# theogf/AugmentedGaussianProcesses.jl

Hardware: AMD Instinct MI355X
Metric: cavi_iters_per_sec (higher is better)
Workload: dtype f64

## Files before the change

augmentedgaussianprocesses.jl_amd/csrc/agp_chol.h:

```cpp
#pragma once
#include "agp_cavi.h"
#include "agp_device.h"

namespace agp {

constexpr int LDP = TILE + 2;
#ifndef AGP_PIVOT_ALG
#define AGP_PIVOT_ALG 0
#endif
constexpr int CHOL_THREADS = 512;

__device__ __forceinline__ double rcp1(double p) {
  double r = __builtin_amdgcn_rcp(p);
  return fma(r, fma(-p, r, 1.0), r);
}
__device__ __forceinline__ double rsqrt1(double p) {
  double y = __builtin_amdgcn_rsq(p);
  const double h = 0.5 * p;
  y = y * fma(-h * y, y, 1.5);
  y = y * fma(-h * y, y, 1.5);
  return y;
}
__device__ __forceinline__ float rsqrt1(float p) {
  float y = __builtin_amdgcn_rsqf(p);
  const float h = 0.5f * p;
  y = y * fmaf(-h * y, y, 1.5f);
  return y;
}
__device__ __forceinline__ float rcp1(float p) {
  float r = __builtin_amdgcn_rcpf(p);
  return fmaf(r, fmaf(-p, r, 1.0f), r);
}

template <typename T, int NT>
__device__ __forceinline__ void load_tile_lds(const T* __restrict__ G, int64_t ld, T* S) {
  typedef typename Mfma<T>::vec_t vec_t;
  constexpr int VEC = Mfma<T>::VEC, NV = TILE / VEC;
#pragma unroll
  for (int v = 0; v < TILE * NV / NT; ++v) {
    int vi = threadIdx.x + v * NT;
    int r = vi / NV, cv = vi % NV;
    vec_t x = *reinterpret_cast<const vec_t*>(G + (int64_t)r * ld + cv * VEC);
#pragma unroll
    for (int e = 0; e < VEC; ++e) S[r * LDP + cv * VEC + e] = x[e];
  }
}

template <typename T>
struct Acc8 {
  typename Mfma<T>::acc_t a[2];
  __device__ __forceinline__ void zero() {
#pragma unroll
    for (int i = 0; i < 2; ++i)
#pragma unroll
      for (int r = 0; r < 4; ++r) a[i][r] = T(0);
  }
};

template <typename T>
__device__ __forceinline__ void mma8(const T* As, const T* Bs, Acc8<T>& acc) {
  const int lane = threadIdx.x & 63, wave = threadIdx.x >> 6, wm = wave >> 2, wn = wave & 3;
#pragma unroll 4
  for (int kk = 0; kk < TILE / 4; ++kk) {
    T a0 = As[(wm * 32 + (lane & 15)) * LDP + kk * 4 + (lane >> 4)];
    T a1 = As[(wm * 32 + 16 + (lane & 15)) * LDP + kk * 4 + (lane >> 4)];
    T b0 = Bs[(wn * 16 + (lane & 15)) * LDP + kk * 4 + (lane >> 4)];
    acc.a[0] = Mfma<T>::mma(a0, b0, acc.a[0]);
    acc.a[1] = Mfma<T>::mma(a1, b0, acc.a[1]);
  }
}

template <typename T>
__device__ __forceinline__ void mma8_sub(const T* As, const T* Bs, Acc8<T>& acc) {
  const int lane = threadIdx.x & 63, wave = threadIdx.x >> 6, wm = wave >> 2, wn = wave & 3;
#pragma unroll 4
  for (int kk = 0; kk < TILE / 4; ++kk) {
    T a0 = -As[(wm * 32 + (lane & 15)) * LDP + kk * 4 + (lane >> 4)];
    T a1 = -As[(wm * 32 + 16 + (lane & 15)) * LDP + kk * 4 + (lane >> 4)];
    T b0 = Bs[(wn * 16 + (lane & 15)) * LDP + kk * 4 + (lane >> 4)];
    acc.a[0] = Mfma<T>::mma(a0, b0, acc.a[0]);
    acc.a[1] = Mfma<T>::mma(a1, b0, acc.a[1]);
  }
}

template <typename T, typename F>
__device__ __forceinline__ void acc8_foreach(Acc8<T>& acc, F f) {
  const int lane = threadIdx.x & 63, wave = threadIdx.x >> 6, wm = wave >> 2, wn = wave & 3;
#pragma unroll
  for (int mi = 0; mi < 2; ++mi)
#pragma unroll
    for (int r = 0; r < 4; ++r) {
      T t = acc.a[mi][r];
      f(wm * 32 + mi * 16 + Mfma<T>::row(lane, r), wn * 16 + (lane & 15), t);
      acc.a[mi][r] = t;
    }
}

template <typename T>
__device__ __forceinline__ void mma_lds64(const T* As, const T* Bs, Acc<T>& acc) {
  const int lane = threadIdx.x & 63, wave = threadIdx.x >> 6, wm = wave >> 1, wn = wave & 1;
#pragma unroll 4
  for (int kk = 0; kk < TILE / 4; ++kk) {
    T a0 = As[(wm * 32 + (lane & 15)) * LDP + kk * 4 + (lane >> 4)];
    T a1 = As[(wm * 32 + 16 + (lane & 15)) * LDP + kk * 4 + (lane >> 4)];
    T b0 = Bs[(wn * 32 + (lane & 15)) * LDP + kk * 4 + (lane >> 4)];
    T b1 = Bs[(wn * 32 + 16 + (lane & 15)) * LDP + kk * 4 + (lane >> 4)];
    acc.a[0][0] = Mfma<T>::mma(a0, b0, acc.a[0][0]);
    acc.a[0][1] = Mfma<T>::mma(a0, b1, acc.a[0][1]);
    acc.a[1][0] = Mfma<T>::mma(a1, b0, acc.a[1][0]);
    acc.a[1][1] = Mfma<T>::mma(a1, b1, acc.a[1][1]);
  }
}

constexpr int SC_ELEMS = 2 * 2 * 4 * TILE;

struct NoHook {
  __device__ __forceinline__ void operator()(int) const {}
};

template <typename T, int J, int NS, typename H, int PIV = 0>
__device__ __forceinline__ void chol_rounds(T (&a)[NS][NS], T (&g)[NS][NS], T* sc, T* piv, const bool act, const int ti,
                                            const int tj, H& hook, const int hbase) {
#pragma unroll 1
  for (int rr = 0; rr < 4; ++rr) {
    const int jj0 = rr * 4, j0 = J * 16 + jj0;
    T* P = sc + (rr & 1) * 4 * TILE;
    T* Mw = sc + 2 * 4 * TILE + (rr & 1) * 4 * TILE;
    if (act && PIV != 4) {
      const int qc = tj - jj0, qr = ti - jj0;
      if (qc >= 0 && qc < 4) {
#pragma unroll
        for (int r = J; r < NS; ++r) {
          T v = a[r][J];
          if (r == J) v = (ti >= jj0) ? v : T(0);
          P[qc * TILE + ti + 16 * r] = v;
        }
      }
      if (qr >= 0 && qr < 4) {
#pragma unroll
        for (int c = 0; c <= J; ++c) Mw[qr * TILE + tj + 16 * c] = g[J][c];
      }
    }
    __syncthreads();
    hook(hbase + rr);
    if (!act) continue;
    if (PIV == 4 || PIV == 5) continue;
    const T d00 = P[j0], d10 = P[j0 + 1], d20 = P[j0 + 2], d30 = P[j0 + 3];
    T d11 = P[TILE + j0 + 1], d21 = P[TILE + j0 + 2], d31 = P[TILE + j0 + 3];
    T d22 = P[2 * TILE + j0 + 2], d32 = P[2 * TILE + j0 + 3], d33 = P[3 * TILE + j0 + 3];
    T r0, r1, r2, r3, l10, l20, l30, l21, l31, l32;
    if (PIV == 2) {
      r0 = r1 = r2 = r3 = T(1);
      l10 = d10;
      l20 = d20;
      l30 = d30;
      l21 = d21;
      l31 = d31;
      l32 = d32;
    } else if (PIV == 1) {
      r0 = rcp1(d00);
      const T n11 = fma(d00, d11, -(d10 * d10)), n21 = fma(d00, d21, -(d20 * d10)), n31 = fma(d00, d31, -(d30 * d10));
      const T n22 = fma(d00, d22, -(d20 * d20)), n32 = fma(d00, d32, -(d30 * d20)), n33 = fma(d00, d33, -(d30 * d30));
      const T rm2 = rcp1(n11);
      const T p22 = fma(n11, n22, -(n21 * n21)) * r0, p32 = fma(n11, n32, -(n31 * n21)) * r0;
      const T p33 = fma(n11, n33, -(n31 * n31)) * r0;
      const T rm3 = rcp1(p22);
      const T m4 = fma(p22, p33, -(p32 * p32)) * rm2;
      const T rm4 = rcp1(m4);
      l10 = d10 * r0;
      l20 = d20 * r0;
      l30 = d30 * r0;
      l21 = n21 * rm2;
      l31 = n31 * rm2;
      l32 = p32 * rm3;
      r1 = d00 * rm2;
      r2 = n11 * rm3;
      r3 = p22 * rm4;
      d11 = n11 * r0;
      d22 = p22 * rm2;
      d33 = m4 * rm3;
    } else {
      r0 = rcp1(d00);
      l10 = d10 * r0;
      l20 = d20 * r0;
      l30 = d30 * r0;
      d11 = fma(-l10, d10, d11);
      d21 = fma(-l20, d10, d21);
      d31 = fma(-l30, d10, d31);
      d22 = fma(-l20, d20, d22);
      d32 = fma(-l30, d20, d32);
      d33 = fma(-l30, d30, d33);
      r1 = rcp1(d11);
      l21 = d21 * r1;
      l31 = d31 * r1;
      d22 = fma(-l21, d21, d22);
      d32 = fma(-l31, d21, d32);
      d33 = fma(-l31, d31, d33);
      r2 = rcp1(d22);
      l32 = d32 * r2;
      d33 = fma(-l32, d32, d33);
// ... 76 lines not shown
  const int ti = (tid & 255) >> 4, tj = tid & 15;
  NoHook nohook;
  T a[4][4], g[4][4];
#pragma unroll
  for (int r = 0; r < 4; ++r)
#pragma unroll
    for (int c = 0; c < 4; ++c) {
      int R = ti + 16 * r, Cc = tj + 16 * c;
      int lo = R >= Cc ? R : Cc, hi = R >= Cc ? Cc : R;
      a[r][c] = bufA[lo * LDP + hi];
      g[r][c] = (R == Cc) ? T(1) : T(0);
    }
  __syncthreads();
  chol_rounds<T, 0, 4, NoHook>(a, g, sc, piv, act, ti, tj, nohook, 0);
  chol_rounds<T, 1, 4, NoHook>(a, g, sc, piv, act, ti, tj, nohook, 0);
  chol_rounds<T, 2, 4, NoHook>(a, g, sc, piv, act, ti, tj, nohook, 0);
  chol_rounds<T, 3, 4, NoHook>(a, g, sc, piv, act, ti, tj, nohook, 0);
  __syncthreads();
  if (tid < TILE) {
    const T p = piv[tid];
    const bool bad = !(p > T(0)) && (col0 + tid) < nvalid;
    const unsigned long long mask = __ballot(bad);
    if (mask != 0ull && tid == 0) {
      int32_t want = (int32_t)(col0 + (__ffsll((long long)mask) - 1) + 1);
      int32_t old = atomicCAS(info, 0, want);
      while (old != 0 && old > want) {
        int32_t prev = atomicCAS(info, old, want);
        if (prev == old) break;
        old = prev;
      }
    }
  }
  if (act) {
    T rsC[4], rsR[4];
#pragma unroll
    for (int q = 0; q < 4; ++q) {
      T pc = piv[tj + 16 * q], pr = piv[ti + 16 * q];
      rsC[q] = rsqrt1(pc > T(0) ? pc : T(1));
      rsR[q] = rsqrt1(pr > T(0) ? pr : T(1));
    }
#pragma unroll
    for (int r = 0; r < 4; ++r)
#pragma unroll
      for (int c = 0; c < 4; ++c) {
        int R = ti + 16 * r, Cc = tj + 16 * c;
        bufA[R * LDP + Cc] = (R >= Cc) ? a[r][c] * rsC[c] : T(0);
        bufB[R * LDP + Cc] = (R >= Cc) ? g[r][c] * rsR[r] : T(0);
      }
  }
  __syncthreads();
}

template <typename T, bool TB, int LDB = LDP>
__device__ __forceinline__ typename Mfma<T>::acc_t mma_blk32(const T* As, const T* Bs, typename Mfma<T>::acc_t acc,
                                                             int wr, int wc, int lane, bool negA) {
#pragma unroll
  for (int kk = 0; kk < 8; ++kk) {
    T a = As[(wr * 16 + (lane & 15)) * LDP + kk * 4 + (lane >> 4)];
    if (negA) a = -a;
    T b = TB ? Bs[(kk * 4 + (lane >> 4)) * LDB + wc * 16 + (lane & 15)]
             : Bs[(wc * 16 + (lane & 15)) * LDB + kk * 4 + (lane >> 4)];
    acc = Mfma<T>::mma(a, b, acc);
  }
  return acc;
}

template <typename T, typename H, int PIV = 0>
__device__ __forceinline__ void elim_block32(T* bufA, T* bufB, int o, T* sc, T* piv, const bool act, const int ti,
                                             const int tj, H& hook) {
  T a[2][2], g[2][2];
#pragma unroll
  for (int r = 0; r < 2; ++r)
#pragma unroll
    for (int c = 0; c < 2; ++c) {
      int R = ti + 16 * r, Cc = tj + 16 * c;
      int lo = R >= Cc ? R : Cc, hi = R >= Cc ? Cc : R;
      a[r][c] = bufA[(o + lo) * LDP + o + hi];
      g[r][c] = (R == Cc) ? T(1) : T(0);
    }
  __syncthreads();
  chol_rounds<T, 0, 2, H, PIV>(a, g, sc, piv + o, act, ti, tj, hook, 0);
  chol_rounds<T, 1, 2, H, PIV>(a, g, sc, piv + o, act, ti, tj, hook, 4);
  __syncthreads();
  if (act) {
    T rsC[2], rsR[2];
#pragma unroll
    for (int q = 0; q < 2; ++q) {
      T pc = piv[o + tj + 16 * q], pr = piv[o + ti + 16 * q];
      rsC[q] = rsqrt1(pc > T(0) ? pc : T(1));
      rsR[q] = rsqrt1(pr > T(0) ? pr : T(1));
    }
#pragma unroll
    for (int r = 0; r < 2; ++r)
#pragma unroll
      for (int c = 0; c < 2; ++c) {
        int R = ti + 16 * r, Cc = tj + 16 * c;
        bufA[(o + R) * LDP + o + Cc] = (R >= Cc) ? a[r][c] * rsC[c] : T(0);
        bufB[(o + R) * LDP + o + Cc] = (R >= Cc) ? g[r][c] * rsR[r] : T(0);
      }
  }
  __syncthreads();
}

template <typename T, typename H, int PIV = AGP_PIVOT_ALG>
__device__ __forceinline__ void factor_diag_tile_2lvl(T* bufA, T* bufB, T* sc, T* piv, int32_t* info, int64_t col0,
                                                      int64_t nvalid, H& hook) {
  const int tid = threadIdx.x;
  const bool act = tid < 256;
  const int ti = (tid & 255) >> 4, tj = tid & 15;
  const int lane = tid & 63, wave = tid >> 6, wr = (wave >> 1) & 1, wc = wave & 1;
  const bool mw = wave < 4;
  typedef typename Mfma<T>::acc_t acc_t;
  NoHook nohook;
  elim_block32<T, NoHook, PIV>(bufA, bufB, 0, sc, piv, act, ti, tj, nohook);
  acc_t acc;
#pragma unroll
  for (int r = 0; r < 4; ++r) acc[r] = T(0);
  if (mw) {
    acc = mma_blk32<T, false>(bufA + 32 * LDP, bufB, acc, wr, wc, lane, false);
#pragma unroll
    for (int r = 0; r < 4; ++r)
      bufB[(32 + wr * 16 + Mfma<T>::row(lane, r)) * LDP + wc * 16 + (lane & 15)] = acc[r];
  } else {
    for (int e = tid - 256; e < 32 * 32; e += (int)blockDim.x - 256) {
      bufA[(e >> 5) * LDP + 32 + (e & 31)] = T(0);
      bufB[(e >> 5) * LDP + 32 + (e & 31)] = T(0);
    }
  }
  __syncthreads();
  if (mw) {
#pragma unroll
    for (int r = 0; r < 4; ++r)
      bufA[(32 + wr * 16 + Mfma<T>::row(lane, r)) * LDP + wc * 16 + (lane & 15)] = acc[r];
    if (wr >= wc) {
#pragma unroll
      for (int r = 0; r < 4; ++r)
        acc[r] = bufA[(32 + wr * 16 + Mfma<T>::row(lane, r)) * LDP + 32 + wc * 16 + (lane & 15)];
      acc = mma_blk32<T, false>(bufB + 32 * LDP, bufB + 32 * LDP, acc, wr, wc, lane, true);
#pragma unroll
      for (int r = 0; r < 4; ++r)
        bufA[(32 + wr * 16 + Mfma<T>::row(lane, r)) * LDP + 32 + wc * 16 + (lane & 15)] = acc[r];
    }
  }
  __syncthreads();
  elim_block32<T, H, PIV>(bufA, bufB, 32, sc, piv, act, ti, tj, hook);
#pragma unroll
  for (int r = 0; r < 4; ++r) acc[r] = T(0);
  if (mw) {
    acc = mma_blk32<T, true>(bufA + 32 * LDP, bufB, acc, wr, wc, lane, false);
#pragma unroll
    for (int r = 0; r < 4; ++r) sc[(wr * 16 + Mfma<T>::row(lane, r)) * 32 + wc * 16 + (lane & 15)] = acc[r];
  }
  __syncthreads();
#pragma unroll
  for (int r = 0; r < 4; ++r) acc[r] = T(0);
  if (mw) {
    acc = mma_blk32<T, true, 32>(bufB + 32 * LDP + 32, sc, acc, wr, wc, lane, true);
#pragma unroll
    for (int r = 0; r < 4; ++r) bufB[(32 + wr * 16 + Mfma<T>::row(lane, r)) * LDP + wc * 16 + (lane & 15)] = acc[r];
  }
  if (blockDim.x <= 256) {
    for (int e = tid; e < 32 * 32; e += blockDim.x) {
      bufA[(e >> 5) * LDP + 32 + (e & 31)] = T(0);
      bufB[(e >> 5) * LDP + 32 + (e & 31)] = T(0);
    }
  }
  if (tid < TILE) {
    const T p = piv[tid];
    const bool bad = !(p > T(0)) && (col0 + tid) < nvalid;
    const unsigned long long mask = __ballot(bad);
    if (mask != 0ull && tid == 0) {
      int32_t want = (int32_t)(col0 + (__ffsll((long long)mask) - 1) + 1);
      int32_t old = atomicCAS(info, 0, want);
      while (old != 0 && old > want) {
        int32_t prev = atomicCAS(info, old, want);
        if (prev == old) break;
        old = prev;
      }
    }
  }
  __syncthreads();
}

template <typename T>
__device__ __forceinline__ void factor_diag_tile_2lvl(T* bufA, T* bufB, T* sc, T* piv, int32_t* info, int64_t col0,
                                                      int64_t nvalid) {
  NoHook nohook;
  factor_diag_tile_2lvl<T, NoHook>(bufA, bufB, sc, piv, info, col0, nvalid, nohook);
}

__device__ __forceinline__ double lane_bcast(double v, int l) {
  const int lo = __builtin_amdgcn_readlane(__double2loint(v), l), hi = __builtin_amdgcn_readlane(__double2hiint(v), l);
  return __hiloint2double(hi, lo);
}
__device__ __forceinline__ float lane_bcast(float v, int l) {
  return __int_as_float(__builtin_amdgcn_readlane(__float_as_int(v), l));
}

template <typename T, bool NN>
__device__ __forceinline__ typename Mfma<T>::acc_t mma16(const T* Ar, const T* sa, const T* Bp, int kend,
                                                         typename Mfma<T>::acc_t acc, bool neg, int lane) {
  const int lr = lane & 15, lk = lane >> 4;
  typename Mfma<T>::acc_t p1;
#pragma unroll
  for (int r = 0; r < 4; ++r) p1[r] = T(0);
#pragma unroll 2
  for (int kk = 0; kk < kend; kk += 8) {
    T a0 = Ar[lr * LDP + kk + lk], a1 = Ar[lr * LDP + kk + 4 + lk];
    if (sa) {
      a0 *= sa[kk + lk];
      a1 *= sa[kk + 4 + lk];
    }
    if (neg) {
      a0 = -a0;
      a1 = -a1;
    }
    const T b0 = NN ? Bp[(kk + lk) * LDP + lr] : Bp[lr * LDP + kk + lk];
    const T b1 = NN ? Bp[(kk + 4 + lk) * LDP + lr] : Bp[lr * LDP + kk + 4 + lk];
    acc = Mfma<T>::mma(a0, b0, acc);
    p1 = Mfma<T>::mma(a1, b1, p1);
  }
#pragma unroll
  for (int r = 0; r < 4; ++r) acc[r] += p1[r];
  return acc;
}

template <typename T>
__device__ __forceinline__ typename Mfma<T>::acc_t acc_load16(const T* P, int lane) {
  typename Mfma<T>::acc_t acc;
#pragma unroll
  for (int r = 0; r < 4; ++r) acc[r] = P[Mfma<T>::row(lane, r) * LDP + (lane & 15)];
  return acc;
}
template <typename T>
__device__ __forceinline__ void acc_store16(T* P, typename Mfma<T>::acc_t acc, int lane) {
#pragma unroll
  for (int r = 0; r < 4; ++r) P[Mfma<T>::row(lane, r) * LDP + (lane & 15)] = acc[r];
}

template <typename T, typename H, int CUT = 0>
__device__ __forceinline__ void factor_diag_tile_panel(T* bufA, T* bufB, T* sc, T* piv, int32_t* info, int64_t col0,
                                                       int64_t nvalid, H& hook) {
  const int tid = threadIdx.x, lane = tid & 63, wave = tid >> 6;
  T* rinv = sc;
  T* rs = sc + TILE;
  typedef typename Mfma<T>::acc_t acc_t;
#pragma unroll 1
  for (int s = 0; s < 4; ++s) {
    const int c0 = 16 * s;
    if (wave == 0 && CUT != 2) {
      T a[16], dv[16], rv[16];
#pragma unroll
      for (int c = 0; c < 16; ++c) a[c] = bufA[lane * LDP + c0 + c];
#pragma unroll
      for (int j = 0; j < 16; ++j) {
        const T d = lane_bcast(a[j], c0 + j);
        const T r = rcp1(d);
        const T l = a[j] * r;
        bufA[lane * LDP + c0 + j] = a[j];
        dv[j] = d;
        rv[j] = r;
#pragma unroll
        for (int c = j + 1; c < 16; ++c) a[c] = fma(-l, lane_bcast(a[j], c0 + c), a[c]);
      }
// ... 651 lines not shown
  __builtin_amdgcn_fence(__ATOMIC_RELEASE, "workgroup");
  __syncthreads();
  if (threadIdx.x == 0) __hip_atomic_fetch_add(sync.done, 1, __ATOMIC_RELAXED, __HIP_MEMORY_SCOPE_AGENT);
}

__global__ void k_handshake(int32_t* mine, const int32_t* theirs, int32_t* ok) {
  if (threadIdx.x != 0) return;
  __hip_atomic_store(mine, 1, __ATOMIC_RELAXED, __HIP_MEMORY_SCOPE_SYSTEM);
  long spins = 0;
  int seen = 0;
  while (!(seen = __hip_atomic_load(theirs, __ATOMIC_RELAXED, __HIP_MEMORY_SCOPE_SYSTEM)) && ++spins < 4000) __builtin_amdgcn_s_sleep(16);
  *ok = seen;
}

__global__ void k_wait_ge(const int32_t* __restrict__ p, int32_t want, int32_t* __restrict__ info) {
  if (threadIdx.x != 0) return;
  long spins = 0;
  while ((int32_t)(__hip_atomic_load(p, __ATOMIC_RELAXED, __HIP_MEMORY_SCOPE_SYSTEM) - want) < 0) {
    __builtin_amdgcn_s_sleep(127);
    if (++spins > (1L << 24)) {
      atomicExch(info, -2);
      break;
    }
  }
}

__global__ void k_wait_ge_fast(const int32_t* __restrict__ p, int32_t want, int32_t* __restrict__ info) {
  if (threadIdx.x != 0) return;
  long spins = 0;
  while ((int32_t)(__hip_atomic_load(p, __ATOMIC_RELAXED, __HIP_MEMORY_SCOPE_SYSTEM) - want) < 0) {
    __builtin_amdgcn_s_sleep(8);
    if (++spins > (1L << 27)) {
      atomicExch(info, -2);
      break;
    }
  }
}

__device__ __forceinline__ void dag_signal(int32_t* flag, int32_t epoch) {
  __builtin_amdgcn_fence(__ATOMIC_RELEASE, "workgroup");
  __syncthreads();
  if (threadIdx.x == 0) __hip_atomic_store(flag, epoch, __ATOMIC_RELAXED, __HIP_MEMORY_SCOPE_AGENT);
}

template <typename T>
__device__ __forceinline__ typename Mfma<T>::acc_t mma_tile16(const T* Ar, const T* Bc, int kend,
                                                              typename Mfma<T>::acc_t acc, bool neg, int lane) {
  const T* pa = Ar + (lane & 15) * LDP + (lane >> 4);
  const T* pb = Bc + (lane & 15) * LDP + (lane >> 4);
  typename Mfma<T>::acc_t p1;
#pragma unroll
  for (int r = 0; r < 4; ++r) p1[r] = T(0);
#pragma unroll 2
  for (int kk = 0; kk < kend / 4; kk += 2) {
    T a0 = pa[kk * 4], a1 = pa[kk * 4 + 4];
    const T b0 = pb[kk * 4], b1 = pb[kk * 4 + 4];
    if (neg) {
      a0 = -a0;
      a1 = -a1;
    }
    acc = Mfma<T>::mma(a0, b0, acc);
    p1 = Mfma<T>::mma(a1, b1, p1);
  }
#pragma unroll
  for (int r = 0; r < 4; ++r) acc[r] += p1[r];
  return acc;
}

template <typename T>
struct ChainPrefetch {
  const T* src;
  T *dT, *dD;
  int* bad;
  const int32_t *f1, *f2;
  int32_t epoch;
  int* ok;
  const T* dgsrc;
  T* gDg;
  const T* lsrc;
  T* gL;
  int ld_i;
  bool coh = false;
  T v[TILE * TILE / 256];
  __device__ __forceinline__ void operator()(int round) {
    int t = (int)threadIdx.x - 256;
    if (t < 0) return;
    if (sizeof(T) == 8) asm volatile("" : "+v"(t));
    if (round < 2) {
      if (dgsrc) {
#pragma unroll
        for (int q = 0; q < TILE * TILE / 512; ++q) {
          const int e = t + (2 * q + round) * 256;
          if (coh) __hip_atomic_store(gDg + e, dgsrc[(e >> 6) * LDP + (e & 63)], __ATOMIC_RELAXED, __HIP_MEMORY_SCOPE_AGENT);
          else gDg[e] = dgsrc[(e >> 6) * LDP + (e & 63)];
        }
      }
      return;
    }
    if (round < 4 && lsrc) {
#pragma unroll
      for (int q = 0; q < TILE * TILE / 512; ++q) {
        const int e = t + (2 * q + (round - 2)) * 256;
        gL[(e >> 6) * ld_i + (e & 63)] = lsrc[(e >> 6) * LDP + (e & 63)];
      }
    }
    if (!src) return;
    if (round == 3) {
      if (t == 0)
        *ok = (__hip_atomic_load(f1, __ATOMIC_RELAXED, __HIP_MEMORY_SCOPE_AGENT) == epoch) &&
              (__hip_atomic_load(f2, __ATOMIC_RELAXED, __HIP_MEMORY_SCOPE_AGENT) == epoch);
      return;
    }
    if (round < 4 || round > 6 || !*ok) return;
    if (round >= 5) {
      T* d = round == 5 ? dT : dD;
#pragma unroll
      for (int q = 0; q < TILE * TILE / 256; ++q) {
        const int e = t + q * 256;
        if (is_sent<T>(v[q])) *bad = 1;
        d[(e >> 6) * LDP + (e & 63)] = v[q];
      }
    }
    if (round <= 5) {
      const T* g = round == 4 ? src : src + TILE * TILE;
#pragma unroll
      for (int q = 0; q < TILE * TILE / 256; ++q)
        v[q] = __hip_atomic_load(g + t + q * 256, __ATOMIC_RELAXED, __HIP_MEMORY_SCOPE_AGENT);
    }
  }
};

typedef unsigned int u32x4 __attribute__((ext_vector_type(4)));
__device__ __forceinline__ u32x4 load16_sc1(const void* p) {
  u32x4 v;
  asm volatile("global_load_dwordx4 %0, %1, off sc1" : "=v"(v) : "v"(p) : "memory");
  return v;
}
__device__ __forceinline__ void wait_vmcnt0() { asm volatile("s_waitcnt vmcnt(0)" ::: "memory"); }
template <typename T>
__device__ __forceinline__ T vec16_elem(u32x4 v, int i);
template <>
__device__ __forceinline__ double vec16_elem<double>(u32x4 v, int i) {
  const unsigned long long u = ((unsigned long long)v[2 * i + 1] << 32) | v[2 * i];
  return __builtin_bit_cast(double, u);
}
template <>
__device__ __forceinline__ float vec16_elem<float>(u32x4 v, int i) {
  return __builtin_bit_cast(float, (unsigned int)v[i]);
}
template <typename T>
__device__ __forceinline__ int pro_slot_off(int tid, int e) {
  constexpr int VEC = 16 / (int)sizeof(T);
  return (e / VEC) * (CHOL_THREADS * VEC) + tid * VEC + (e % VEC);
}

template <typename T>
struct EpiArgs {
  int on = 0;
  int64_t B = 0;
  int nslices = 0;
  const T* pk = nullptr;
  int64_t ldp = 0;
  T kdiag = T(0);
  const T* kd_ptr = nullptr;
  int use_kt = 0;
  T jitter = T(0), rho = T(0);
  LikParams<T> lp{};
  const T* y = nullptr;
  const int64_t* idx = nullptr;
  T *Kt = nullptr, *muf = nullptr, *varf = nullptr, *cb = nullptr, *theta = nullptr, *r = nullptr, *w = nullptr;
  int* flags = nullptr;
  const T* lam = nullptr;
  T* gamma = nullptr;
};

template <typename T>
struct ProArgs {
  const T* kap = nullptr;
  int64_t ldk = 0, Kdim = 0;
  const T* w = nullptr;
  const T* r = nullptr;
  T* eta2 = nullptr;
  const T* Kinv = nullptr;
  int64_t ldm = 0;
  T* eta1 = nullptr;
  const T* kinv_mu0 = nullptr;
  T lr = T(0);
  T* HS = nullptr;
  int32_t* sflags = nullptr;
  T* fill = nullptr;
  int64_t fill_n = 0;
  int32_t nfill = 0;
  const T* packed = nullptr;
// ... 54 lines not shown
    __syncthreads();
  }
}

constexpr int ARRIVE_STRIDE = 16;
__device__ __forceinline__ void pro_arrival_gate(const int32_t* arrive, int g, int32_t want, int32_t* info) {
  if (threadIdx.x == 0) {
    long spins = 0;
    while ((int32_t)(__hip_atomic_load(arrive + g * ARRIVE_STRIDE, __ATOMIC_RELAXED, __HIP_MEMORY_SCOPE_AGENT) - want) < 0) {
      __builtin_amdgcn_s_sleep(8);
      if (++spins > (1L << 23)) {
        atomicExch(info, -4);
        break;
      }
    }
  }
  __syncthreads();
  __builtin_amdgcn_fence(__ATOMIC_ACQUIRE, "agent");
}

constexpr int PRO_NEAR = 4;
__host__ __device__ __forceinline__ int64_t pro_nhelp(int64_t nt, int64_t c, int ks, int kf) {
  const int64_t ntc = nt - c, nn = ntc < PRO_NEAR ? ntc : PRO_NEAR;
  return nn * (kf - 1) + (ntc - nn) * (ks - 1);
}
template <typename T>
__device__ __forceinline__ void pro_slice(const T* __restrict__ kap, int64_t ldk, const T* __restrict__ w, int64_t R0, int64_t c0,
                                          int64_t q0, int64_t q1, T* sm, Acc8<T>& acc) {
  constexpr int Q = TILE * TILE / CHOL_THREADS;
  const int r = threadIdx.x & 63, kb = threadIdx.x >> 6;
  const bool dg = R0 == c0;
  T va[Q], vb[Q], wv[Q];
  auto ldg = [&](int64_t qc) {
    const T* __restrict__ p = kap + (qc * TILE) * ldk;
#pragma unroll
    for (int q = 0; q < Q; ++q) {
      const int k = kb + 8 * q;
      va[q] = p[k * ldk + R0 + r];
      vb[q] = dg ? T(0) : p[k * ldk + c0 + r];
      wv[q] = w[qc * TILE + k];
    }
  };
  if (q0 < q1) ldg(q0);
  int cur = 0;
  for (int64_t qc = q0; qc < q1; ++qc) {
    T* As = sm + cur * 2 * TILE * LDP;
    T* Bs = As + TILE * LDP;
#pragma unroll
    for (int q = 0; q < Q; ++q) {
      const int k = kb + 8 * q;
      As[r * LDP + k] = va[q] * wv[q];
      Bs[r * LDP + k] = dg ? va[q] : vb[q];
    }
    __syncthreads();
    if (qc + 1 < q1) ldg(qc + 1);
    mma8<T>(As, Bs, acc);
    cur ^= 1;
  }
  __syncthreads();
}

constexpr long long CHAIN_GO_TICKS = 4LL * 100000000LL;
#ifndef AGP_TILES_WAVES_F64
#define AGP_TILES_WAVES_F64 4
#endif
#ifndef AGP_TILES_WAVES_F32
#define AGP_TILES_WAVES_F32 6
#endif
template <typename T, int ROLE, bool PRO>
constexpr int dag_min_waves() {
  return ROLE != 2 ? 1 : PRO ? (sizeof(T) == 8 ? 2 : 4) : (sizeof(T) == 8 ? AGP_TILES_WAVES_F64 : AGP_TILES_WAVES_F32);
}
template <typename T>
struct ProdArgs {
  T* out = nullptr;
  int64_t ld = 0;
  int64_t base = 0;
  T* fill = nullptr;
  int64_t fill_n = 0;
  double* ld_out = nullptr;
  int32_t* status = nullptr;
};

constexpr int STRACE_SLOTS = 8192, STRACE_XPUB = 600, STRACE_EXT = 1100, STRACE_FILL0 = 1400, STRACE_FILL1 = 1500, STRACE_WG0 = 2048,
              STRACE_WG1 = 4096, STRACE_MAXWG = 2048, STRACE_SAFE0 = 6144, STRACE_SAFE1 = 6400;
#ifdef AGP_STEP_TRACE
struct StraceExit {
  unsigned long long* p;
  __device__ ~StraceExit() {
    if (p && threadIdx.x == 0) *p = wall_clock64();
  }
};
#define STRACE(i) \
  if (PRO && ROLE == 0 && trace && threadIdx.x == 0) trace[i] = wall_clock64()
#else
#define STRACE(i)
#endif

template <typename T, bool FUSED, bool BATCH = false, bool TRACE = false, bool STEP = false, bool PRO = false, int ROLE = 0>
__global__ __launch_bounds__(CHOL_THREADS, (dag_min_waves<T, ROLE, PRO>()))
void k_chol_dag(CholBatch<T> bt, int nb, int64_t fstride, int64_t ld, int64_t ldx,
                                                           int64_t lde, int64_t ne, int64_t nt,
                                                           int32_t* __restrict__ info, int64_t nvalid, int32_t* flags,
                                                           int32_t epoch, unsigned long long* trace, T* H, int64_t hstride,
                                                           int64_t nx_, const T* __restrict__ erow, int opts, DagSync sync,
                                                           ProArgs<T> pro = ProArgs<T>{}, EpiArgs<T> epi = EpiArgs<T>{},
                                                           ProdArgs<T> prod = ProdArgs<T>{}) {
  static_assert(!PRO || (FUSED && !BATCH), "the prologue exists for single-problem launches with a chain workgroup only");
  static_assert(ROLE == 0 || (FUSED && STEP && !TRACE), "the split launch exists for the CAVI step's launches");
  const int64_t nx = STEP ? 0 : nx_;
  const int write_x = STEP ? 0 : (opts & 1);
  const bool store_l = STEP ? false : (opts & 2) != 0;
  const int prob = BATCH ? (int)(blockIdx.x % (unsigned)nb) : 0;
  const int64_t bidx = BATCH ? (int64_t)(blockIdx.x / (unsigned)nb) : (int64_t)blockIdx.x;
  T* A = bt.A[prob];
  T* X = bt.X[prob];
  T* __restrict__ Dg = bt.Dg[prob];
  T* E = bt.E[prob];
  if (BATCH) erow = bt.R[prob];
  flags += prob * fstride;
  constexpr int64_t SLOT = TILE * TILE;
  T* HX = H + prob * hstride;
  T* HP = HX + nt * SLOT;
  T* HL = HP + 2 * nt * SLOT;
  __shared__ __attribute__((aligned(16))) T sm[((FUSED && ROLE != 2) || PRO ? 4 : 2) * TILE * LDP];
  __shared__ __attribute__((aligned(16))) T sc[(ROLE == 2 && !PRO) ? TILE : SC_ELEMS];
  __shared__ T piv[TILE];
  __shared__ int wait_ok, pf_ok, pf_bad;
  if (ROLE == 1) {
    if (threadIdx.x == 0) {
      wait_ok = 1;
      if (sync.here) __hip_atomic_fetch_add(sync.here, 1, __ATOMIC_RELAXED, __HIP_MEMORY_SCOPE_SYSTEM);
      unsigned spins = 0;
      const long long t0 = (long long)wall_clock64();
      while (sync.go) {
        const int32_t d = (int32_t)(__hip_atomic_load(sync.go, __ATOMIC_RELAXED, __HIP_MEMORY_SCOPE_SYSTEM) - sync.go_val);
        if (d == 0) break;
        if (d > 0) {
          wait_ok = 0;
          break;
        }
        __builtin_amdgcn_s_sleep(4);
        if ((++spins & 1023u) == 0 && (long long)wall_clock64() - t0 > CHAIN_GO_TICKS) {
          atomicExch(info, -1);
          wait_ok = 0;
#ifdef AGP_DEBUG_PTRS
          atomicAdd(&agp_dag_diag[5], 1ull);
#endif
          break;
        }
      }
    }
    __syncthreads();
    if (!wait_ok) {
      chain_count_out(sync);
      return;
    }
    __builtin_amdgcn_fence(__ATOMIC_ACQUIRE, "agent");
  }
  T* bufA = sm;
  T* bufB = sm + TILE * LDP;
  const int tid = threadIdx.x;
#ifdef AGP_STEP_TRACE
  StraceExit strace_exit{(PRO && ROLE == 0 && trace && bidx < STRACE_MAXWG) ? trace + STRACE_WG1 + bidx : nullptr};
  if (bidx < STRACE_MAXWG) STRACE(STRACE_WG0 + bidx);
#endif
// ... 251 lines not shown
      acc8_foreach<T>(acc, [&](int r, int cc, T& val) {
        pro.eta2[(R * TILE + r) * pro.ldm + c0 + cc] = val;
        pro.eta2[(c0 + cc) * pro.ldm + R * TILE + r] = val;
        val *= T(-2);
      });
    }
    PRO_TS(tsb + 4);
  } else if (idr) {
    const bool on_diag = (R - nt - ne) == c;
    acc8_foreach<T>(acc, [&](int r, int cc, T& val) { val = (on_diag && r == cc) ? T(1) : T(0); });
  } else if (PRO && ext && R == nt + ne - 1) {
    if (pro.tred && pro.arrive) pro_arrival_gate(pro.arrive, 0, pro.arrive_want, info);
    const int col = tid & 63, grp = tid >> 6;
    T s0 = T(0), s1 = T(0), s2 = T(0), s3 = T(0);
    int64_t k = grp;
    for (; k + 24 < pro.Kdim; k += 32) {
      const T a0 = pro.kap[k * pro.ldk + c0 + col], a1 = pro.kap[(k + 8) * pro.ldk + c0 + col];
      const T a2 = pro.kap[(k + 16) * pro.ldk + c0 + col], a3 = pro.kap[(k + 24) * pro.ldk + c0 + col];
      s0 += a0 * pro.r[k];
      s1 += a1 * pro.r[k + 8];
      s2 += a2 * pro.r[k + 16];
      s3 += a3 * pro.r[k + 24];
    }
    for (; k < pro.Kdim; k += 8) s0 += pro.kap[k * pro.ldk + c0 + col] * pro.r[k];
    sc[grp * TILE + col] = (s0 + s1) + (s2 + s3);
    __syncthreads();
    if (grp == 0) {
      T t = T(0);
#pragma unroll
      for (int q = 0; q < CHOL_THREADS / 64; ++q) t += sc[q * TILE + col];
      if (pro.tred) t = pro.tred[c0 + col];
      T e = pro.eta1[c0 + col];
      e += pro.lr * (t + (pro.kinv_mu0 ? pro.kinv_mu0[c0 + col] : T(0)) - e);
      pro.eta1[c0 + col] = e;
      sc[CHOL_THREADS + col] = e;
    }
    __syncthreads();
    acc8_foreach<T>(acc, [&](int r, int cc, T& val) { val = r == 0 ? sc[CHOL_THREADS + cc] : T(0); });
    __syncthreads();
  } else if (erow && ext && R == nt + ne - 1) {
    acc8_foreach<T>(acc, [&](int r, int cc, T& val) { val = r == 0 ? erow[c0 + cc] : T(0); });
  } else {
    acc8_foreach<T>(acc, [&](int r, int cc, T& val) { val = rowp[r * ldr + c0 + cc]; });
  }
  if (PRO && ROLE == 2 && chain) {
    T* park = HP + SLOT;
    acc8_foreach<T>(acc, [&](int r, int cc, T& val) {
      __hip_atomic_store(park + r * TILE + cc, val, __ATOMIC_RELAXED, __HIP_MEMORY_SCOPE_AGENT);
    });
    dag_signal(pre2, epoch);
    return;
  }
  if (ROLE != 2 && chain) {
    if (PRO && ROLE == 1) {
      if (!dag_wait(pre2, nullptr, epoch, abortf, info, &wait_ok)) {
        chain_count_out(sync);
        return;
      }
      load_tile_lds_hv<T>(HP + SLOT, bufA);
    } else {
      acc8_foreach<T>(acc, [&](int r, int cc, T& val) { bufA[r * LDP + cc] = val; });
    }
    __syncthreads();
    T* bufC = sm + (FUSED ? 2 : 0) * TILE * LDP;
    T* bufD = sm + (FUSED ? 3 : 0) * TILE * LDP;
    for (int64_t k = 0; k < nt; ++k) {
      const int64_t k0 = k * TILE;
      T* trow = A + (k + 1) * TILE * ld;
      ChainPrefetch<T> pf;
      pf.src = k + 1 < nt ? HP + 2 * (k + 1) * SLOT : nullptr;
      pf.bad = &pf_bad;
      pf.dT = bufC;
      pf.dD = bufD;
      pf.f1 = pre1 + (k + 1) * DAG_FS;
      pf.f2 = pre2 + (k + 1) * DAG_FS;
      pf.epoch = epoch;
      pf.ok = &pf_ok;
      pf.dgsrc = k >= 1 ? bufD : nullptr;
      pf.gDg = Dg + (k - 1) * TILE * TILE;
      pf.lsrc = (k >= 1 && store_l) ? bufC : nullptr;
      pf.gL = A + k0 * ld + (k0 - TILE);
      pf.ld_i = (int)ld;
      pf.coh = ROLE == 1;
      if (tid == 0) pf_ok = pf_bad = 0;
      factor_diag_tile_2lvl<T, ChainPrefetch<T>>(bufA, bufB, sc, piv, info, k0, nvalid, pf);
      DAG_TRC(k, 2);
      PRO_TS(512 + k);
      {
        T xv[TILE * TILE / CHOL_THREADS];
        int tl = tid;
        asm volatile("" : "+v"(tl));
#pragma unroll
        for (int q = 0; q < TILE * TILE / CHOL_THREADS; ++q) {
          const int e = tl + q * CHOL_THREADS;
          xv[q] = bufB[(e >> 6) * LDP + (e & 63)];
        }
#pragma unroll
        for (int q = 0; q < TILE * TILE / CHOL_THREADS; ++q) {
          const int e = tl + q * CHOL_THREADS;
          __hip_atomic_store(HX + k * SLOT + e, xv[q], __ATOMIC_RELAXED, __HIP_MEMORY_SCOPE_AGENT);
          if (write_x) X[(k0 + (e >> 6)) * ldx + k0 + (e & 63)] = xv[q];
        }
      }
      if (k + 1 == nt) {
        for (int e = tid; e < TILE * TILE; e += CHOL_THREADS) {
          if (ROLE == 1) __hip_atomic_store(Dg + k * TILE * TILE + e, bufA[(e >> 6) * LDP + (e & 63)], __ATOMIC_RELAXED, __HIP_MEMORY_SCOPE_AGENT);
          else Dg[k * TILE * TILE + e] = bufA[(e >> 6) * LDP + (e & 63)];
        }
        dag_signal(xready + k * DAG_FS, epoch);
        DAG_TRC(k, 3);
        STRACE(STRACE_XPUB);
        if (ROLE == 1) chain_count_out(sync);
        return;
      }
      const bool late_feed = !pf_ok || pf_bad;
      if (late_feed) {
        dag_signal(xready + k * DAG_FS, epoch);
        DAG_TRC(k, 3);
        if (!dag_wait(pf.f1, pf.f2, epoch, abortf, info, &wait_ok)) {
          if (ROLE == 1) chain_count_out(sync);
          return;
        }
        load_tiles_lds_hv2<T>(HP + 2 * (k + 1) * SLOT, bufC, HP + (2 * (k + 1) + 1) * SLOT, bufD);
        __syncthreads();
      }
      if (TRACE && tid == 0) trace[chain_slot(k + 1, nt, ne, nx) * 8 + 7] = (unsigned long long)pf_ok;
      DAG_TRC(k + 1, 4);
      typedef typename Mfma<T>::acc_t acc_t;
      const int lane = tid & 63, wave = tid >> 6;
      {
        const int ri = wave >> 1, cA = (wave & 1) ? 2 : 3, cB = 3 - cA;
        acc_t oa, ob;
#pragma unroll
        for (int r = 0; r < 4; ++r) oa[r] = ob[r] = T(0);
        oa = mma_tile16<T>(bufC + 16 * ri * LDP, bufB + 16 * cA * LDP, 16 * (cA + 1), oa, false, lane);
        ob = mma_tile16<T>(bufC + 16 * ri * LDP, bufB + 16 * cB * LDP, 16 * (cB + 1), ob, false, lane);
        if (!late_feed) {
          dag_signal(xready + k * DAG_FS, epoch);
          DAG_TRC(k, 3);
        } else {
          __syncthreads();
        }
#pragma unroll
        for (int r = 0; r < 4; ++r) {
          const int row = 16 * ri + Mfma<T>::row(lane, r);
          bufC[row * LDP + 16 * cA + (lane & 15)] = oa[r];
          bufC[row * LDP + 16 * cB + (lane & 15)] = ob[r];
          T* hl = HL + ((k + 1) * nt + k) * SLOT + row * TILE + (lane & 15);
          __hip_atomic_store(hl + 16 * cA, oa[r], __ATOMIC_RELAXED, __HIP_MEMORY_SCOPE_AGENT);
          __hip_atomic_store(hl + 16 * cB, ob[r], __ATOMIC_RELAXED, __HIP_MEMORY_SCOPE_AGENT);
        }
      }
      __syncthreads();
      DAG_TRC(k + 1, 5);
      {
        const int ti_[10] = {0, 1, 1, 2, 2, 2, 3, 3, 3, 3}, tj_[10] = {0, 0, 1, 0, 1, 2, 0, 1, 2, 3};
#pragma unroll
        for (int rep = 0; rep < 2; ++rep) {
          const int tl = rep == 0 ? 2 + wave : wave;
          if (rep == 1 && wave >= 2) break;
          int i2 = 0, j2 = 0;
#pragma unroll
          for (int q = 0; q < 10; ++q)
            if (q == tl) {
              i2 = ti_[q];
              j2 = tj_[q];
// ... 210 lines not shown
```

Measured before the change: 3259.

## Overlap L21*X11 glue MMA with second diagonal elimination via idle waves

Moves the L21·X11 product that followed the second 32x32 elimination block into a hook run by the otherwise idle waves 4-7 during a chosen elimination round. The accumulator is written to scratch once the rounds finish, which removes a serial MMA phase and one block barrier from the diagonal-tile factorization. It also drops a redundant zero-fill branch, hardcodes the thread stride, and adds optional step-trace timestamps. The upper waves now carry both the prefetch work and the MMA, which may add register pressure and contention in the rounds.

Measured after the change: 3289 (median of 6 runs). Within noise of the previous version (+0.9%).

```diff
diff --git a/augmentedgaussianprocesses.jl_amd/csrc/agp_chol.h b/augmentedgaussianprocesses.jl_amd/csrc/agp_chol.h
--- a/augmentedgaussianprocesses.jl_amd/csrc/agp_chol.h
+++ b/augmentedgaussianprocesses.jl_amd/csrc/agp_chol.h
@@ -7,6 +7,9 @@
 constexpr int LDP = TILE + 2;
 #ifndef AGP_PIVOT_ALG
 #define AGP_PIVOT_ALG 0
+#endif
+#ifndef AGP_GLUE_ROUND
+#define AGP_GLUE_ROUND 2
 #endif
 constexpr int CHOL_THREADS = 512;
 
@@ -115,7 +118,10 @@
 constexpr int SC_ELEMS = 2 * 2 * 4 * TILE;
 
 struct NoHook {
+  static constexpr int glue_round = 0;
   __device__ __forceinline__ void operator()(int) const {}
+  __device__ __forceinline__ void after_rounds() const {}
+  __device__ __forceinline__ void stamp(int) const {}
 };
 
 template <typename T, int J, int NS, typename H, int PIV = 0>
@@ -358,6 +364,7 @@
   chol_rounds<T, 0, 2, H, PIV>(a, g, sc, piv + o, act, ti, tj, hook, 0);
   chol_rounds<T, 1, 2, H, PIV>(a, g, sc, piv + o, act, ti, tj, hook, 4);
   __syncthreads();
+  hook.after_rounds();
   if (act) {
     T rsC[2], rsR[2];
 #pragma unroll
@@ -377,6 +384,31 @@
   }
   __syncthreads();
 }
+
+template <typename T, typename H>
+struct GlueP {
+  typedef typename Mfma<T>::acc_t acc_t;
+  H& inner;
+  const T *L21, *X11;
+  T* sc;
+  acc_t acc;
+  __device__ __forceinline__ GlueP(H& h, const T* l21, const T* x11, T* s) : inner(h), L21(l21), X11(x11), sc(s) {
+#pragma unroll
+    for (int r = 0; r < 4; ++r) acc[r] = T(0);
+  }
+  __device__ __forceinline__ void operator()(int round) {
+    inner(round);
+    const int tid = threadIdx.x, lane = tid & 63, wave = tid >> 6, wr = (wave >> 1) & 1, wc = wave & 1;
+    if (round == H::glue_round && wave >= 4) acc = mma_blk32<T, true>(L21, X11, acc, wr, wc, lane, false);
+  }
+  __device__ __forceinline__ void after_rounds() {
+    const int tid = threadIdx.x, lane = tid & 63, wave = tid >> 6, wr = (wave >> 1) & 1, wc = wave & 1;
+    if (wave >= 4) {
+#pragma unroll
+      for (int r = 0; r < 4; ++r) sc[(wr * 16 + Mfma<T>::row(lane, r)) * 32 + wc * 16 + (lane & 15)] = acc[r];
+    }
+  }
+};
 
 template <typename T, typename H, int PIV = AGP_PIVOT_ALG>
 __device__ __forceinline__ void factor_diag_tile_2lvl(T* bufA, T* bufB, T* sc, T* piv, int32_t* info, int64_t col0,
@@ -388,7 +420,9 @@
   const bool mw = wave < 4;
   typedef typename Mfma<T>::acc_t acc_t;
   NoHook nohook;
+  hook.stamp(0);
   elim_block32<T, NoHook, PIV>(bufA, bufB, 0, sc, piv, act, ti, tj, nohook);
+  hook.stamp(1);
   acc_t acc;
 #pragma unroll
   for (int r = 0; r < 4; ++r) acc[r] = T(0);
@@ -398,12 +432,13 @@
     for (int r = 0; r < 4; ++r)
       bufB[(32 + wr * 16 + Mfma<T>::row(lane, r)) * LDP + wc * 16 + (lane & 15)] = acc[r];
   } else {
-    for (int e = tid - 256; e < 32 * 32; e += (int)blockDim.x - 256) {
+    for (int e = tid - 256; e < 32 * 32; e += CHOL_THREADS - 256) {
       bufA[(e >> 5) * LDP + 32 + (e & 31)] = T(0);
       bufB[(e >> 5) * LDP + 32 + (e & 31)] = T(0);
     }
   }
   __syncthreads();
+  hook.stamp(2);
   if (mw) {
 #pragma unroll
     for (int r = 0; r < 4; ++r)
@@ -419,27 +454,16 @@
     }
   }
   __syncthreads();
-  elim_block32<T, H, PIV>(bufA, bufB, 32, sc, piv, act, ti, tj, hook);
-#pragma unroll
-  for (int r = 0; r < 4; ++r) acc[r] = T(0);
-  if (mw) {
-    acc = mma_blk32<T, true>(bufA + 32 * LDP, bufB, acc, wr, wc, lane, false);
-#pragma unroll
-    for (int r = 0; r < 4; ++r) sc[(wr * 16 + Mfma<T>::row(lane, r)) * 32 + wc * 16 + (lane & 15)] = acc[r];
-  }
-  __syncthreads();
+  hook.stamp(3);
+  GlueP<T, H> glue(hook, bufA + 32 * LDP, bufB, sc);
+  elim_block32<T, GlueP<T, H>, PIV>(bufA, bufB, 32, sc, piv, act, ti, tj, glue);
+  hook.stamp(4);
 #pragma unroll
   for (int r = 0; r < 4; ++r) acc[r] = T(0);
   if (mw) {
     acc = mma_blk32<T, true, 32>(bufB + 32 * LDP + 32, sc, acc, wr, wc, lane, true);
 #pragma unroll
     for (int r = 0; r < 4; ++r) bufB[(32 + wr * 16 + Mfma<T>::row(lane, r)) * LDP + wc * 16 + (lane & 15)] = acc[r];
-  }
-  if (blockDim.x <= 256) {
-    for (int e = tid; e < 32 * 32; e += blockDim.x) {
-      bufA[(e >> 5) * LDP + 32 + (e & 31)] = T(0);
-      bufB[(e >> 5) * LDP + 32 + (e & 31)] = T(0);
-    }
   }
   if (tid < TILE) {
     const T p = piv[tid];
@@ -456,6 +480,7 @@
     }
   }
   __syncthreads();
+  hook.stamp(6);
 }
 
 template <typename T>
@@ -1273,7 +1298,17 @@
   int ld_i;
   bool coh = false;
   T v[TILE * TILE / 256];
+  static constexpr int glue_round = AGP_GLUE_ROUND;
+#ifdef AGP_STEP_TRACE
+  unsigned long long* ts = nullptr;
+  __device__ __forceinline__ void stamp(int i) const {
+    if (ts && threadIdx.x == 0) ts[i] = wall_clock64();
+  }
+#else
+  __device__ __forceinline__ void stamp(int) const {}
+#endif
   __device__ __forceinline__ void operator()(int round) {
+    stamp(16 + round);
     int t = (int)threadIdx.x - 256;
     if (t < 0) return;
     if (sizeof(T) == 8) asm volatile("" : "+v"(t));
@@ -1297,9 +1332,17 @@
     }
     if (!src) return;
     if (round == 3) {
-      if (t == 0)
-        *ok = (__hip_atomic_load(f1, __ATOMIC_RELAXED, __HIP_MEMORY_SCOPE_AGENT) == epoch) &&
-              (__hip_atomic_load(f2, __ATOMIC_RELAXED, __HIP_MEMORY_SCOPE_AGENT) == epoch);
+      if (t == 0) {
+#ifdef AGP_STEP_TRACE
+        if (ts) ts[8] = wall_clock64();
+#endif
+        const int32_t s1 = __hip_atomic_load(f1, __ATOMIC_RELAXED, __HIP_MEMORY_SCOPE_AGENT);
+        const int32_t s2 = __hip_atomic_load(f2, __ATOMIC_RELAXED, __HIP_MEMORY_SCOPE_AGENT);
+        *ok = (int)(s1 == epoch) & (int)(s2 == epoch);
+#ifdef AGP_STEP_TRACE
+        if (ts) ts[9] = wall_clock64();
+#endif
+      }
       return;
     }
     if (round < 4 || round > 6 || !*ok) return;
@@ -1520,6 +1563,7 @@
   int32_t* status = nullptr;
 };
 
+constexpr int STRACE_TILE = 1600, STRACE_MAXCOL = 14;
 constexpr int STRACE_SLOTS = 8192, STRACE_XPUB = 600, STRACE_EXT = 1100, STRACE_FILL0 = 1400, STRACE_FILL1 = 1500, STRACE_WG0 = 2048,
               STRACE_WG1 = 4096, STRACE_MAXWG = 2048, STRACE_SAFE0 = 6144, STRACE_SAFE1 = 6400;
 #ifdef AGP_STEP_TRACE
@@ -1937,6 +1981,9 @@
       pf.gL = A + k0 * ld + (k0 - TILE);
       pf.ld_i = (int)ld;
       pf.coh = ROLE == 1;
+#ifdef AGP_STEP_TRACE
+      pf.ts = (PRO && trace && k < STRACE_MAXCOL) ? trace + STRACE_TILE + 32 * k : nullptr;
+#endif
       if (tid == 0) pf_ok = pf_bad = 0;
       factor_diag_tile_2lvl<T, ChainPrefetch<T>>(bufA, bufB, sc, piv, info, k0, nvalid, pf);
       DAG_TRC(k, 2);
```
